# cmp-nct/ggllm.cpp

Hardware: NVIDIA B200
Metric: falcon40b_q4_k_decode_tokens_per_s (higher is better)
Workload: dtype int8 x int4 block dots (dp4a), fp32 accumulate; f32 KV/attention

## Files before the change

### ggllm.cpp_b200/csrc/bwtest.cu

```cuda
#include "common.cuh"
__global__ void __launch_bounds__(256) read_kernel(const uint4 * __restrict__ p, size_t n, int unroll_dummy, unsigned * out) {
    unsigned acc = 0;
    const size_t stride = (size_t) gridDim.x * blockDim.x;
    size_t i = (size_t) blockIdx.x * blockDim.x + threadIdx.x;
    for (; i + 7 * stride < n; i += 8 * stride) {
        uint4 v[8];
#pragma unroll
        for (int u = 0; u < 8; u++) v[u] = ldg_stream_v4(p + i + u * stride);
#pragma unroll
        for (int u = 0; u < 8; u++) acc += v[u].x ^ v[u].y ^ v[u].z ^ v[u].w;
    }
    for (; i < n; i += stride) { const uint4 v = ldg_stream_v4(p + i); acc += v.x ^ v.y ^ v.z ^ v.w; }
    if (acc == 0x12345678u && unroll_dummy) *out = acc;
}
extern "C" float b200_read_bandwidth_gbs(size_t bytes, int ctas_per_sm) {
    void * p = nullptr; unsigned * o = nullptr;
    B200_CUDA_CHECK(cudaMalloc(&p, bytes)); B200_CUDA_CHECK(cudaMalloc(&o, 4));
    B200_CUDA_CHECK(cudaMemset(p, 1, bytes));
    int dev, sms; cudaGetDevice(&dev); cudaDeviceGetAttribute(&sms, cudaDevAttrMultiProcessorCount, dev);
    cudaEvent_t e0, e1; cudaEventCreate(&e0); cudaEventCreate(&e1);
    float best = 0.f;
    for (int it = 0; it < 6; it++) {
        cudaEventRecord(e0);
        read_kernel<<<sms * ctas_per_sm, 256>>>((const uint4 *) p, bytes / 16, 0, o);
        cudaEventRecord(e1); cudaEventSynchronize(e1);
        float ms; cudaEventElapsedTime(&ms, e0, e1);
        const float g = (float) (bytes / 1e6 / ms);
        if (it > 0 && g > best) best = g;
    }
    cudaFree(p); cudaFree(o);
    return best;
}
```

### ggllm.cpp_b200/csrc/common.cuh

```cuda
#pragma once
#include <cuda_runtime.h>
#include <cuda_fp16.h>
#include <cstdint>
#include <cstdio>
#include <cstdlib>

#define B200_CUDA_CHECK(expr)                                                                        \
    do {                                                                                             \
        cudaError_t err_ = (expr);                                                                   \
        if (err_ != cudaSuccess) {                                                                   \
            fprintf(stderr, "b200: CUDA error %d (%s) at %s:%d: %s\n", (int) err_,                   \
                    cudaGetErrorString(err_), __FILE__, __LINE__, #expr);                            \
            exit(1);                                                                                 \
        }                                                                                            \
    } while (0)

#define B200_ASSERT(x)                                                                               \
    do {                                                                                             \
        if (!(x)) {                                                                                  \
            fprintf(stderr, "B200_ASSERT: %s:%d: %s\n", __FILE__, __LINE__, #x);                     \
            abort();                                                                                 \
        }                                                                                            \
    } while (0)

enum : int {
    T_F32 = 0, T_F16 = 1, T_Q4_0 = 2, T_Q4_1 = 3, T_Q5_0 = 6, T_Q5_1 = 7, T_Q8_0 = 8, T_Q8_1 = 9,
    T_Q2_K = 10, T_Q3_K = 11, T_Q4_K = 12, T_Q5_K = 13, T_Q6_K = 14, T_Q8_K = 15,
};

static inline size_t round_up(size_t v, size_t a) { return (v + a - 1) / a * a; }

#define B200_CARVEOUT 25

#ifdef __CUDACC__

__device__ __forceinline__ uint4 ldg_stream_v4(const void * p) {
    uint4 r;
    asm volatile("ld.global.nc.L1::no_allocate.v4.u32 {%0,%1,%2,%3}, [%4];"
                 : "=r"(r.x), "=r"(r.y), "=r"(r.z), "=r"(r.w) : "l"(p));
    return r;
}
__device__ __forceinline__ uint2 ldg_stream_v2(const void * p) {
    uint2 r;
    asm volatile("ld.global.nc.L1::no_allocate.v2.u32 {%0,%1}, [%2];" : "=r"(r.x), "=r"(r.y) : "l"(p));
    return r;
}
__device__ __forceinline__ uint32_t ldg_stream_u32(const void * p) {
    uint32_t r;
    asm volatile("ld.global.nc.L1::no_allocate.u32 %0, [%1];" : "=r"(r) : "l"(p));
    return r;
}
__device__ __forceinline__ uint4 ldg_v4(const void * p) { return __ldg(reinterpret_cast<const uint4 *>(p)); }
__device__ __forceinline__ uint32_t ldg_u32(const void * p) { return __ldg(reinterpret_cast<const uint32_t *>(p)); }
__device__ __forceinline__ uint16_t ldg_u16(const void * p) { return __ldg(reinterpret_cast<const uint16_t *>(p)); }

__device__ __forceinline__ float f16_bits_to_f32(uint16_t h) { return __half2float(__ushort_as_half(h)); }
__device__ __forceinline__ uint16_t f32_to_f16_bits(float f) { return __half_as_ushort(__float2half_rn(f)); }

__device__ __forceinline__ float warp_sum(float v) {
#pragma unroll
    for (int o = 16; o > 0; o >>= 1) v += __shfl_xor_sync(0xffffffffu, v, o);
    return v;
}
__device__ __forceinline__ float warp_max(float v) {
#pragma unroll
    for (int o = 16; o > 0; o >>= 1) v = fmaxf(v, __shfl_xor_sync(0xffffffffu, v, o));
    return v;
}
__device__ __forceinline__ double warp_sum_d(double v) {
#pragma unroll
    for (int o = 16; o > 0; o >>= 1) v += __shfl_xor_sync(0xffffffffu, v, o);
    return v;
}

__device__ __forceinline__ int dp4a_ss(int a, int b, int c) { return __dp4a(a, b, c); }
__device__ __forceinline__ int dp4a_us(unsigned a, int b, int c) {
    int d;
    asm("dp4a.u32.s32 %0, %1, %2, %3;" : "=r"(d) : "r"(a), "r"(b), "r"(c));
    return d;
}

__device__ __forceinline__ uint32_t smem_u32(const void * p) { return (uint32_t) __cvta_generic_to_shared(p); }
__device__ __forceinline__ void mbar_init(uint64_t * bar, uint32_t count) {
    asm volatile("mbarrier.init.shared::cta.b64 [%0], %1;" :: "r"(smem_u32(bar)), "r"(count));
}
__device__ __forceinline__ void mbar_fence_init() { asm volatile("fence.mbarrier_init.release.cluster;" ::: "memory"); }
__device__ __forceinline__ void mbar_expect_tx(uint64_t * bar, uint32_t bytes) {
    asm volatile("mbarrier.arrive.expect_tx.shared::cta.b64 _, [%0], %1;" :: "r"(smem_u32(bar)), "r"(bytes) : "memory");
}
__device__ __forceinline__ void mbar_wait(uint64_t * bar, uint32_t phase) {
    asm volatile(
        "{\n\t.reg .pred p;\n\t"
        "WAIT_%=:\n\t"
        "mbarrier.try_wait.parity.shared::cta.b64 p, [%0], %1;\n\t"
        "@p bra DONE_%=;\n\t"
        "bra WAIT_%=;\n\t"
        "DONE_%=:\n\t}"
        :: "r"(smem_u32(bar)), "r"(phase) : "memory");
}
__device__ __forceinline__ void tma_load_1d(void * smem_dst, const void * gmem_src, uint32_t bytes, uint64_t * bar) {
    asm volatile("cp.async.bulk.shared::cluster.global.mbarrier::complete_tx::bytes [%0], [%1], %2, [%3];"
                 :: "r"(smem_u32(smem_dst)), "l"(gmem_src), "r"(bytes), "r"(smem_u32(bar)) : "memory");
}

__device__ __forceinline__ unsigned long long gtimer() { unsigned long long t; asm volatile("mov.u64 %0, %globaltimer;" : "=l"(t)); return t; }
__device__ __forceinline__ void trace_begin(unsigned long long * slot) { if (slot && threadIdx.x == 0) atomicMin(slot, gtimer()); }
__device__ __forceinline__ void trace_end(unsigned long long * slot) { if (slot && threadIdx.x == 0) atomicMax(slot + 1, gtimer()); }

#endif

unsigned long long * b200_trace_slot(const char * name);
```

### ggllm.cpp_b200/csrc/kernels.h

```cpp
#pragma once
#include "formats.cuh"

size_t wplanes_layout(WPlanes & W, int type, int K, int M);
void   wplanes_upload(WPlanes & W, int type, int K, int M, const void * host_raw, cudaStream_t stream);
void   wplanes_from_device_raw(WPlanes & W, int type, int K, int M, const void * dev_raw, cudaStream_t stream);
void   wplanes_alloc_random(WPlanes & W, int type, int K, int M, uint64_t seed, cudaStream_t stream);
void   launch_repack_rows(const WPlanes & W, const void * stage_dev, int64_t row0, int64_t nrows, cudaStream_t stream);
void   wplanes_free(WPlanes & W);
void   launch_dequant_rows(const WPlanes & W, const int32_t * rows_dev, int nrows, float * dst, int64_t dst_stride, cudaStream_t stream);

size_t actq_bytes(int act_type, int K, int N);
void   actq_bind(ActQ & A, int act_type, int K, int N, void * base);
void   launch_quantize_act(const float * x, int64_t x_stride, const ActQ & A, cudaStream_t stream);
void   launch_actq_to_f16(const ActQ & A, __half * dst, int64_t dst_stride, cudaStream_t stream);

enum { EPI_NONE = 0, EPI_GELU = 1, EPI_ADD2 = 2 };
struct MmvEpilogue { int kind; const float * r1; const float * r2;
    const ActQ * qout; unsigned * qctr;
    int late_wait; };
void   launch_mmv(const WPlanes & W, const ActQ & A, float * y, int64_t y_stride, MmvEpilogue epi, cudaStream_t stream);
void   launch_mmv_f(const WPlanes & W, const float * x, int64_t x_stride, int N, float * y, int64_t y_stride, cudaStream_t stream);

struct FastX {
    int mode;
    int N;
    ActQ A;
    const float * x; int64_t x_stride;
    const float * ra, * rb;
    const float * gamma, * beta;
    float * x_out;
    int l2_dist;
};
bool   launch_mmv_fast_x(const WPlanes & W, const FastX & X, float * y, int64_t y_stride, MmvEpilogue e, cudaStream_t stream);
bool   mmv_fast_supports(int wtype, int K, int mode);
bool   mmv_fast_fills_sm(const WPlanes & W);
void   launch_layernorm(const float * x, int64_t x_stride, const float * g, const float * b, float * y, int64_t y_stride,
                        int n, int rows, cudaStream_t stream);
void   launch_argmax(const float * x, int n, int32_t * out_a, int32_t * out_b, cudaStream_t stream);
void   launch_argmax_hist(const float * x, int n, int32_t * out, int32_t * hist, int * step, cudaStream_t stream);
void   launch_layernorm_q(float * x, int64_t x_stride, const float * ra, const float * rb, int64_t r_stride,
                          const float * g1, const float * b1, const ActQ * A1,
                          const float * g2, const float * b2, const ActQ * A2, int n, int rows, cudaStream_t stream);
void   launch_gelu(const float * x, float * y, int64_t n, cudaStream_t stream);
void   launch_f32_to_f16(const float * x, __half * y, int64_t n, cudaStream_t stream);
void   launch_add(const float * a, const float * b, float * y, int64_t n, cudaStream_t stream);
void   launch_add3(const float * a, const float * b, const float * c, float * y, int64_t n, cudaStream_t stream);
void   launch_mul_bcast(const float * a, const float * b, float * y, int64_t n, int64_t nb, cudaStream_t stream);
void   launch_add_bcast(const float * a, const float * b, float * y, int64_t n, int64_t nb, cudaStream_t stream);
void   launch_scale(const float * a, float s, float * y, int64_t n, cudaStream_t stream);
struct RopeParams { int n_past; int head_dim; float theta_scale; };
float  rope_theta_scale_host(int head_dim, int n_ctx_rope, int dynamic_mode, float ntk_alpha, int freq_base);
void   launch_rope_neox(float * x, int n_tok, int n_head, int head_dim, int64_t tok_stride, int n_past, const int * n_past_dev,
                        float theta_scale, cudaStream_t stream);

struct AttnParams {
    int n_head, n_head_kv, head_dim;
    int n_tok;
    int n_past;
    const int * n_past_dev;
    int n_ctx;
    int64_t qkv_stride;
    unsigned long long * trace;
    const ActQ * qout;
    __half * k16; __half * vt16;
    int fuse_rope; float rope_theta_scale;
    int long_ctx;
};
int    attention_long_threshold();
void   launch_rope_kv_append(float * qkv, float * k_cache, float * v_cache, const AttnParams & p, float theta_scale, cudaStream_t stream);
int    launch_attention(const float * qkv, const float * k_cache, const float * v_cache, float * out, int64_t out_stride,
                        const AttnParams & p, float * scratch, cudaStream_t stream);
size_t attention_scratch_bytes(const AttnParams & p);
bool   launch_attention_ws(const float * qkv, float * out, int64_t out_stride, const AttnParams & p, cudaStream_t stream);
int    attention_ctx_pad(int n_ctx);
size_t attention_shadow_halves(int n_head_kv, int n_ctx);
void   launch_kv_shadow_refresh(const float * k_cache, const float * v_cache, __half * k16, __half * vt16, int n_head_kv, int n_ctx, int pos, int n, cudaStream_t stream);
size_t attention_prefill_scratch_bytes(int n_head, int n_tok, int T);
void   launch_attention_prefill(const float * qkv, const float * k_cache, const float * v_cache, float * out, int64_t out_stride,
                                const AttnParams & p, float * scratch, cudaStream_t stream);

void   launch_mmq_gemm(const WPlanes & W, const __half * X, int64_t x_stride, int N, float * Y, int64_t y_stride,
                       int epi_gelu, void * workspace, size_t workspace_bytes, cudaStream_t stream);
size_t mmq_gemm_workspace_bytes(const WPlanes & W, int N);

#define B200_SAMPLER_MAX_WINDOW 256
struct SamplerParams { int top_k; float top_p; float temp; float repeat_penalty; };
struct SamplerState;
SamplerState * sampler_state_alloc();
void   sampler_state_free(SamplerState * s);
void   launch_sampler_init(SamplerState * s, uint32_t seed, const int32_t * window_dev, int n, int cap, cudaStream_t stream);
void   launch_sample(const float * logits, int n_vocab, const SamplerParams & p, SamplerState * st, float * work, int32_t * out, int32_t * hist, int * step, cudaStream_t stream);

struct b200_falcon;
bool   falcon_adopt_matrix(b200_falcon * f, const char * ggcc_name, const WPlanes & W);
int    falcon_eval_begin(b200_falcon * f, const int32_t * tokens, int n_tokens, int n_past, int n_ctx_rope, int all_logits);
void   falcon_eval_finish(b200_falcon * f, float * logits);
```

### ggllm.cpp_b200/csrc/mmv_fast.cu

```cuda
#include "kernels.h"

#include "mmv_fast.cuh"

template <int TYPE, int NT, int J, int D, int MODE>
__device__ __forceinline__ void mmv_body(const WPlanes & W, const FastX & X, float * __restrict__ y, int64_t y_stride, const Epi & epi,
                                         const int cta, const int nctas, const int n, uint8_t * smem) {
    using T = FX<TYPE>;
    constexpr int NW = NT / 32;
    uint64_t * bar = reinterpret_cast<uint64_t *>(smem);
    float * partial = reinterpret_cast<float *>(smem + 16);
    double * red = reinterpret_cast<double *>(smem + 16 + 2 * NW * 4 * 4);
    int8_t * xq = reinterpret_cast<int8_t *>(smem + ((16 + 2 * NW * 4 * 4 + NW * 8 + 15) & ~15));
    const int tid = threadIdx.x, lane = tid & 31, warp = tid >> 5;
    const int P = W.nb * T::PPB;
    const ActQ & A = X.A;

    trace_begin(epi.trace);
    if (tid == 0 && MODE == 0) { mbar_init(bar, 1); mbar_fence_init(); }
    const int per = W.M / nctas, rem = W.M % nctas;
    const int row0 = cta * per + min(cta, rem), row1 = row0 + per + (cta < rem ? 1 : 0);
    const int nrows = row1 - row0;

    int gidx[J]; bool valid[J];
    WP wp[J];
    int aux[J];
#pragma unroll
    for (int j = 0; j < J; j++) { const int g = j * NT + tid; valid[j] = g < P; gidx[j] = valid[j] ? g : P - 1; wp[j] = T::wp(W, gidx[j]); aux[j] = piece_aux<TYPE>(gidx[j]); }

    typename T::WR w[D][J];
    ring_fill<TYPE, J, D>(w, wp, row0, row1);
    const L2PF pf = l2pf_of(W, X.l2_dist);
    if (pf.dist > 0 && tid == 0) l2_prefetch_rows(pf, min(row0 + D, row1), min(row0 + D + pf.dist, row1));

    if (!epi.late_wait) asm volatile("griddepcontrol.wait;" ::: "memory");
    typename T::XR xr[J];
    if (MODE == 0) {
        if (tid == 0) {
            mbar_expect_tx(bar, (uint32_t) W.K);
            tma_load_1d(xq, A.q + (size_t) n * W.K, (uint32_t) W.K, bar);
        }
        __syncthreads();
        mbar_wait(bar, 0);
#pragma unroll
        for (int j = 0; j < J; j++) xr[j] = valid[j] ? T::load_x(xq, A, n, gidx[j]) : zero_xr<TYPE>();
    } else if constexpr (T::HAS_PROLOGUE_QUANT) {
        const float * xrow = X.x + (size_t) n * X.x_stride;
        float mean = 0.f, scale = 1.f;
#pragma unroll
        for (int j = 0; j < J; j++) {
            int ea, eb; T::seg(gidx[j], ea, eb);
            float v[32];
#pragma unroll
            for (int i = 0; i < 4; i++) {
                const float4 a = *reinterpret_cast<const float4 *>(xrow + ea + 4 * i), b = *reinterpret_cast<const float4 *>(xrow + eb + 4 * i);
                v[4 * i] = a.x; v[4 * i + 1] = a.y; v[4 * i + 2] = a.z; v[4 * i + 3] = a.w;
                v[16 + 4 * i] = b.x; v[17 + 4 * i] = b.y; v[18 + 4 * i] = b.z; v[19 + 4 * i] = b.w;
            }
            if (MODE == 2 && J == 1) {
                if (X.ra) {
                    const float * ra = X.ra + (size_t) n * X.x_stride, * rb = X.rb + (size_t) n * X.x_stride;
#pragma unroll
                    for (int i = 0; i < 16; i++) { v[i] = __fadd_rn(__fadd_rn(ra[ea + i], rb[ea + i]), v[i]); v[16 + i] = __fadd_rn(__fadd_rn(ra[eb + i], rb[eb + i]), v[16 + i]); }
                }
                if (X.x_out && cta == 0 && valid[j]) {
                    float * xo = X.x_out + (size_t) n * X.x_stride;
#pragma unroll
                    for (int i = 0; i < 16; i++) { xo[ea + i] = v[i]; xo[eb + i] = v[16 + i]; }
                }
                double s = 0.0;
                if (valid[j]) {
#pragma unroll
                    for (int i = 0; i < 32; i++) s += (double) v[i];
                }
                s = warp_sum_d(s);
                if (lane == 0) red[warp] = s;
                __syncthreads();
                double t = 0.0;
#pragma unroll
                for (int wi = 0; wi < NW; wi++) t += red[wi];
                mean = (float) (t / W.K);
                __syncthreads();
                double s2 = 0.0;
                if (valid[j]) {
#pragma unroll
                    for (int i = 0; i < 32; i++) { const float c = __fsub_rn(v[i], mean); s2 += (double) __fmul_rn(c, c); }
                }
                s2 = warp_sum_d(s2);
                if (lane == 0) red[warp] = s2;
                __syncthreads();
                t = 0.0;
#pragma unroll
                for (int wi = 0; wi < NW; wi++) t += red[wi];
                scale = __fdiv_rn(1.0f, __fsqrt_rn(__fadd_rn((float) (t / W.K), 1e-5f)));
#pragma unroll
                for (int i = 0; i < 16; i++) {
                    v[i] = __fadd_rn(__fmul_rn(__fmul_rn(__fsub_rn(v[i], mean), scale), X.gamma[ea + i]), X.beta[ea + i]);
                    v[16 + i] = __fadd_rn(__fmul_rn(__fmul_rn(__fsub_rn(v[16 + i], mean), scale), X.gamma[eb + i]), X.beta[eb + i]);
                }
            }
            if (!valid[j]) {
#pragma unroll
                for (int i = 0; i < 32; i++) v[i] = 0.f;
            }
            xr[j] = T::quant_x(v, gidx[j], lane);
        }
        __syncthreads();
    }

    int gcount = 0;
    const int ekind = epi.kind; const float * r1p = epi.r1, * r2p = epi.r2;
    ring_run<TYPE, NT, J, D, false>(w, wp, row0, row1, wp, 0, 0, xr, aux, partial, gcount, 0, tid,
        [&](int row, float v) {
            if (ekind == EPI_GELU) v = gelu_lut(v);
            else if (ekind == EPI_ADD2) v = (v + r1p[(size_t) n * y_stride + row]) + r2p[(size_t) n * y_stride + row];
            y[(size_t) n * y_stride + row] = v;
        },
        [&]() { asm volatile("griddepcontrol.launch_dependents;" ::: "memory"); }, pf);
    if (epi.late_wait) asm volatile("griddepcontrol.wait;" ::: "memory");
    if (epi.qctr) {
        __shared__ int s_do;
        __threadfence();
        __syncthreads();
        if (nrows > 0) {
            for (int b = row0 >> 8; b <= (row1 - 1) >> 8; b++) {
                if (tid == 0) {
                    const unsigned cnt = (unsigned) (min(row1, (b + 1) << 8) - max(row0, b << 8));
                    const unsigned old = atomicAdd(epi.qctr + b, cnt);
                    s_do = old + cnt == 256u;
                    if (s_do) epi.qctr[b] = 0;
                }
                __syncthreads();
                if (s_do && warp == 0) {
                    __threadfence();
                    const float * src = y + (size_t) n * y_stride + (b << 8) + lane * 8;
                    const float4 p = __ldcg(reinterpret_cast<const float4 *>(src)), q = __ldcg(reinterpret_cast<const float4 *>(src) + 1);
                    const float v[8] = { p.x, p.y, p.z, p.w, q.x, q.y, q.z, q.w };
                    if (epi.qA.type == T_Q8_K) quantize_chunk8<T_Q8_K>(v, lane, epi.qA, n, (b << 8) + lane * 8);
                    else quantize_chunk8<T_Q8_0>(v, lane, epi.qA, n, (b << 8) + lane * 8);
                }
                __syncthreads();
            }
        }
    }
    trace_end(epi.trace);
}

template <int TYPE, int NT, int J, int D, int MODE>
__global__ void __launch_bounds__(NT) __maxnreg__(NT <= 256 ? 96 : 128) mmv_fast_kernel(const WPlanes W, const FastX X, float * __restrict__ y, int64_t y_stride, const Epi epi) {
    extern __shared__ __align__(16) uint8_t smem[];
    mmv_body<TYPE, NT, J, D, MODE>(W, X, y, y_stride, epi, (int) blockIdx.x, (int) gridDim.x, (int) blockIdx.y, smem);
}

static int fast_num_sms() {
    static int n = 0;
    if (!n) { int dev; B200_CUDA_CHECK(cudaGetDevice(&dev)); B200_CUDA_CHECK(cudaDeviceGetAttribute(&n, cudaDevAttrMultiProcessorCount, dev)); }
    return n;
}

template <int TYPE, int NT, int J, int D, int MODE>
static void launch_mode(const WPlanes & W, const FastX & X, float * y, int64_t y_stride, Epi epi, cudaStream_t stream) {
    const size_t smem = ((16 + 2 * (NT / 32) * 4 * 4 + (NT / 32) * 8 + 15) & ~15) + (size_t) ((W.K + 15) & ~15);
    static bool set = false;
    if (!set) { B200_CUDA_CHECK(cudaFuncSetAttribute(mmv_fast_kernel<TYPE, NT, J, D, MODE>, cudaFuncAttributeMaxDynamicSharedMemorySize, 100 * 1024));
        B200_CUDA_CHECK(cudaFuncSetAttribute(mmv_fast_kernel<TYPE, NT, J, D, MODE>, cudaFuncAttributePreferredSharedMemoryCarveout, B200_CARVEOUT)); set = true; }
    int ctas = fast_num_sms() * (NT == 128 ? 4 : NT == 160 || NT == 192 ? 3 : NT == 256 ? 2 : 1);
    if (ctas > (W.M + 3) / 4) ctas = (W.M + 3) / 4;
    cudaLaunchConfig_t cfg{};
    cfg.gridDim = dim3((unsigned) ctas, (unsigned) X.N); cfg.blockDim = dim3(NT); cfg.dynamicSmemBytes = smem; cfg.stream = stream;
    cudaLaunchAttribute attr[1];
    attr[0].id = cudaLaunchAttributeProgrammaticStreamSerialization;
    attr[0].val.programmaticStreamSerializationAllowed = 1;
    cfg.attrs = attr; cfg.numAttrs = getenv("B200_NO_PDL") ? 0 : 1;
    B200_CUDA_CHECK(cudaLaunchKernelEx(&cfg, mmv_fast_kernel<TYPE, NT, J, D, MODE>, W, X, y, y_stride, epi));
}
template <int TYPE, int NT, int J, int D>
static void launch_cfg(const WPlanes & W, const FastX & X, float * y, int64_t y_stride, Epi epi, cudaStream_t stream) {
    if (X.mode == 0) launch_mode<TYPE, NT, J, D, 0>(W, X, y, y_stride, epi, stream);
    else if constexpr (FX<TYPE>::HAS_PROLOGUE_QUANT) {
        if (X.mode == 1) launch_mode<TYPE, NT, J, D, 1>(W, X, y, y_stride, epi, stream);
        else if (J == 1) launch_mode<TYPE, NT, J, D, J == 1 ? 2 : 1>(W, X, y, y_stride, epi, stream);
        else B200_ASSERT(!"mmv_fast: LayerNorm prologue needs J == 1");
    } else B200_ASSERT(!"mmv_fast: this weight type takes quantised activations only (mode 0)");
}

template <int TYPE>
static bool launch_type(const WPlanes & W, const FastX & X, float * y, int64_t y_stride, Epi epi, cudaStream_t stream) {
    const int P = W.nb * FX<TYPE>::PPB;
    if (W.K > 64 * 1024) return false;
    if (X.mode == 2 && P > 512) return false;
    constexpr int D1 = FX<TYPE>::D256;
    if (P <= 128 && D1 == 4) launch_cfg<TYPE, 128, 1, D1>(W, X, y, y_stride, epi, stream);
    else if (P > 128 && P <= 160 && D1 == 8 && !getenv("B200_NO_NT160")) launch_cfg<TYPE, 160, 1, D1>(W, X, y, y_stride, epi, stream);
    else if (P <= 256) launch_cfg<TYPE, 256, 1, D1>(W, X, y, y_stride, epi, stream);
    else if (P > 256 && P <= 512 && D1 == 8 && X.mode == 0 && !getenv("B200_NO_NT256J2")) launch_cfg<TYPE, 256, 2, D1 / 2>(W, X, y, y_stride, epi, stream);
    else if (P <= 512) launch_cfg<TYPE, 512, 1, D1>(W, X, y, y_stride, epi, stream);
    else if (P > 512 && P <= 576 && D1 == 8 && X.mode == 0 && !getenv("B200_NO_NT192")) launch_cfg<TYPE, 192, 3, 2>(W, X, y, y_stride, epi, stream);
    else if (P <= 1024) launch_cfg<TYPE, 512, 2, D1 / 2>(W, X, y, y_stride, epi, stream);
    else if (P <= 2048 && D1 == 8) launch_cfg<TYPE, 512, 4, 2>(W, X, y, y_stride, epi, stream);
    else return false;
    return true;
}

bool launch_mmv_fast_x(const WPlanes & W, const FastX & X, float * y, int64_t y_stride, MmvEpilogue e, cudaStream_t stream) {
    const char * nm = W.M > 40000 ? "mmv_lmhead" : W.K > 16384 ? "mmv_down" : W.M > 16384 ? "mmv_up" : W.M > 8192 ? "mmv_qkv" : "mmv_wo";
    Epi epi = { e.kind, e.r1, e.r2, b200_trace_slot(nm), ActQ{}, nullptr, getenv("B200_NO_LATE_WAIT") ? 0 : e.late_wait };
    if (e.qout && e.qctr) {
        B200_ASSERT(X.N == 1 && W.M % 256 == 0 && e.qout->K == W.M && (e.qout->type == T_Q8_K || e.qout->type == T_Q8_0));
        epi.qA = *e.qout; epi.qctr = e.qctr;
    }
    static int dist_bytes = -1;
    if (dist_bytes < 0) { const char * s = getenv("B200_L2PF_KB"); dist_bytes = (s ? atoi(s) : 0) * 1024; }
    FastX Xp = X;
    Xp.l2_dist = W.stride[0] ? (int) (dist_bytes / W.stride[0]) : 0;
    switch (W.type) {
        case T_Q4_K: return launch_type<T_Q4_K>(W, Xp, y, y_stride, epi, stream);
        case T_Q4_0: return launch_type<T_Q4_0>(W, Xp, y, y_stride, epi, stream);
        case T_Q3_K: return X.mode == 0 && !getenv("B200_Q3K_GENERIC") && launch_type<T_Q3_K>(W, Xp, y, y_stride, epi, stream);
    }
    return false;
}
bool mmv_fast_supports(int wtype, int K, int mode) {
    if (wtype != T_Q4_K && wtype != T_Q4_0) return false;
    const int P = wtype == T_Q4_K ? K / 32 : K / 32;
    return K <= 64 * 1024 && P <= (mode == 2 ? 512 : 2048);
}
bool mmv_fast_fills_sm(const WPlanes & W) {
    if ((W.type != T_Q4_K && W.type != T_Q4_0) || getenv("B200_NO_NT192")) return false;
    const int P = W.K / 32;
    return P > 512 && P <= 576;
}
bool launch_mmv_fast(const WPlanes & W, const ActQ & A, float * y, int64_t y_stride, MmvEpilogue e, cudaStream_t stream) {
    FastX X{}; X.mode = 0; X.A = A; X.N = A.N;
    return launch_mmv_fast_x(W, X, y, y_stride, e, stream);
}
```

### ggllm.cpp_b200/csrc/mmv_fast.cuh

```cuda
#pragma once
#include "kernels.h"
#include "actquant.cuh"

struct Epi { int kind; const float * r1; const float * r2; unsigned long long * trace; ActQ qA; unsigned * qctr; int late_wait; };


__device__ __forceinline__ int dot16(const uint32_t w0, const uint32_t w1, const uint32_t w2, const uint32_t w3, const uint4 x) {
    int s = dp4a_us(w0, (int) x.x, 0); s = dp4a_us(w1, (int) x.y, s); s = dp4a_us(w2, (int) x.z, s); return dp4a_us(w3, (int) x.w, s);
}
__device__ __forceinline__ int dp2a_lo_su(int pair16, uint32_t bytes) { int d; asm("dp2a.lo.s32.u32 %0, %1, %2, %3;" : "=r"(d) : "r"(pair16), "r"(bytes), "r"(0)); return d; }
__device__ __forceinline__ int dp2a_hi_su(int pair16, uint32_t bytes) { int d; asm("dp2a.hi.s32.u32 %0, %1, %2, %3;" : "=r"(d) : "r"(pair16), "r"(bytes), "r"(0)); return d; }
__device__ __forceinline__ int dp2a_lo_ss(int pair16, uint32_t bytes, int c) { int d; asm("dp2a.lo.s32.s32 %0, %1, %2, %3;" : "=r"(d) : "r"(pair16), "r"(bytes), "r"(c)); return d; }
__device__ __forceinline__ int dp2a_hi_ss(int pair16, uint32_t bytes, int c) { int d; asm("dp2a.hi.s32.s32 %0, %1, %2, %3;" : "=r"(d) : "r"(pair16), "r"(bytes), "r"(c)); return d; }
__device__ __forceinline__ float gelu_lut(float v) {
    const float f = __half2float(__float2half_rn(v));
    const float g = 0.5f * f * (1.0f + tanhf(0.79788456080286535587989211986876f * f * (1.0f + 0.044715f * f * f)));
    return __half2float(__float2half_rn(g));
}

struct WP { const uint8_t * b0, * b1, * b2, * b3; uint32_t s0, s1, s2, s3; };
__device__ __forceinline__ const uint8_t * opaque_ptr(const uint8_t * p) { unsigned long long v = (unsigned long long) p; asm volatile("" : "+l"(v)); return (const uint8_t *) v; }

template <int TYPE> struct FX;

template <> struct FX<T_Q4_K> {
    static constexpr int PPB = 8;
    static constexpr bool HAS_PROLOGUE_QUANT = true;
    static constexpr int D256 = 8;
    struct XR { uint4 xl, xh; int bs; float xd; };
    struct WR { uint4 q; uint32_t sm, dd; };
    __device__ static XR load_x(const int8_t * xq, const ActQ & A, int n, int g) {
        const int b = g >> 3, pc = g & 7, p = pc >> 1, half = pc & 1;
        XR r;
        const int e0 = b * 256 + 64 * p + 16 * half;
        r.xl = *reinterpret_cast<const uint4 *>(xq + e0);
        r.xh = *reinterpret_cast<const uint4 *>(xq + e0 + 32);
        const int16_t * bs = A.bs + (size_t) n * (A.K / 16) + b * 16 + 4 * p + half;
        r.bs = ((int) bs[0] & 0xffff) | ((int) bs[2] << 16);
        r.xd = A.d[(size_t) n * (A.K / 256) + b];
        return r;
    }
    __device__ static void seg(int g, int & ea, int & eb) { const int b = g >> 3, pc = g & 7; ea = b * 256 + 64 * (pc >> 1) + 16 * (pc & 1); eb = ea + 32; }
    __device__ static XR quant_x(const float (&v)[32], int g, int lane) {
        int ea, eb; seg(g, ea, eb);
        float amax = 0.f, vmax = 0.f; int imax = 0;
#pragma unroll
        for (int i = 0; i < 32; i++) { const float ax = fabsf(v[i]); const int idx = (i < 16 ? ea : eb - 16) + i; if (ax > amax || (ax == amax && ax > 0.f && idx < imax)) { amax = ax; vmax = v[i]; imax = idx; } }
#pragma unroll
        for (int o = 1; o < 8; o <<= 1) {
            const float oa = __shfl_xor_sync(0xffffffffu, amax, o), ov = __shfl_xor_sync(0xffffffffu, vmax, o);
            const int oi = __shfl_xor_sync(0xffffffffu, imax, o);
            if (oa > amax || (oa == amax && oi < imax)) { amax = oa; vmax = ov; imax = oi; }
        }
        XR r;
        const bool zero = amax == 0.f;
        const float iscale = zero ? 0.f : __fdiv_rn(-128.f, vmax);
        r.xd = zero ? 0.f : __fdiv_rn(1.f, iscale);
        int s0 = 0, s1 = 0;
        uint32_t w[8];
#pragma unroll
        for (int i = 0; i < 8; i++) {
            uint32_t pk = 0;
#pragma unroll
            for (int k = 0; k < 4; k++) {
                const int q = zero ? 0 : min(127, __float2int_rn(__fmul_rn(iscale, v[4 * i + k])));
                if (i < 4) s0 += q; else s1 += q;
                pk |= (uint32_t) (q & 0xff) << (8 * k);
            }
            w[i] = pk;
        }
        r.xl = make_uint4(w[0], w[1], w[2], w[3]); r.xh = make_uint4(w[4], w[5], w[6], w[7]);
        r.bs = (s0 & 0xffff) | (s1 << 16);
        (void) lane;
        return r;
    }
    __device__ static WP wp(const WPlanes & W, int g) {
        WP r; r.b0 = opaque_ptr(W.p[0] + (size_t) g * 16); r.b1 = opaque_ptr(W.p[1] + (size_t) (g >> 1) * 4); r.b2 = opaque_ptr(W.p[2] + (size_t) (g >> 3) * 4);
        r.s0 = W.stride[0]; r.s1 = W.stride[1]; r.s2 = W.stride[2];
        return r;
    }
    __device__ static WR load_w(const WP & p, uint32_t row) {
        WR r;
        r.q = ldg_stream_v4(p.b0 + (uint64_t) row * p.s0);
        r.sm = ldg_u32(p.b1 + (uint64_t) row * p.s1);
        r.dd = ldg_u32(p.b2 + (uint64_t) row * p.s2);
        return r;
    }
    __device__ static float dot(const WR & w, const XR & x) {
        const int il = dot16(w.q.x & 0x0F0F0F0F, w.q.y & 0x0F0F0F0F, w.q.z & 0x0F0F0F0F, w.q.w & 0x0F0F0F0F, x.xl);
        const int ih = dot16(w.q.x & 0xF0F0F0F0, w.q.y & 0xF0F0F0F0, w.q.z & 0xF0F0F0F0, w.q.w & 0xF0F0F0F0, x.xh) >> 4;
        const int isum = dp2a_lo_su((il & 0xffff) | (ih << 16), w.sm);
        const int msum = dp2a_hi_su(x.bs, w.sm);
        const float2 dm = __half22float2(*reinterpret_cast<const __half2 *>(&w.dd));
        return (dm.x * x.xd) * (float) isum - (dm.y * x.xd) * (float) msum;
    }
};

template <> struct FX<T_Q4_0> {
    static constexpr int PPB = 1;
    static constexpr bool HAS_PROLOGUE_QUANT = true;
    static constexpr int D256 = 8;
    struct XR { uint4 xl, xh; int bs; float xd; };
    struct WR { uint4 q; uint32_t d; };
    __device__ static XR load_x(const int8_t * xq, const ActQ & A, int n, int g) {
        XR r;
        r.xl = *reinterpret_cast<const uint4 *>(xq + g * 32);
        r.xh = *reinterpret_cast<const uint4 *>(xq + g * 32 + 16);
        r.bs = A.bs[(size_t) n * (A.K / 32) + g];
        r.xd = A.d[(size_t) n * (A.K / 32) + g];
        return r;
    }
    __device__ static void seg(int g, int & ea, int & eb) { ea = g * 32; eb = ea + 16; }
    __device__ static XR quant_x(const float (&v)[32], int, int) {
        float amax = 0.f;
#pragma unroll
        for (int i = 0; i < 32; i++) amax = fmaxf(amax, fabsf(v[i]));
        const float id = amax != 0.f ? __fdiv_rn(127.f, amax) : 0.f;
        XR r;
        r.xd = __half2float(__float2half_rn(__fdiv_rn(amax, 127.f)));
        int s = 0;
        uint32_t w[8];
#pragma unroll
        for (int i = 0; i < 8; i++) {
            uint32_t pk = 0;
#pragma unroll
            for (int k = 0; k < 4; k++) { const int q = __float2int_rn(__fmul_rn(v[4 * i + k], id)); s += q; pk |= (uint32_t) (q & 0xff) << (8 * k); }
            w[i] = pk;
        }
        r.xl = make_uint4(w[0], w[1], w[2], w[3]); r.xh = make_uint4(w[4], w[5], w[6], w[7]);
        r.bs = s;
        return r;
    }
    __device__ static WP wp(const WPlanes & W, int g) {
        WP r; r.b0 = opaque_ptr(W.p[0] + (size_t) g * 16); r.b1 = opaque_ptr(W.p[1] + (size_t) g * 2); r.b2 = nullptr;
        r.s0 = W.stride[0]; r.s1 = W.stride[1]; r.s2 = 0;
        return r;
    }
    __device__ static WR load_w(const WP & p, uint32_t row) {
        WR r;
        r.q = ldg_stream_v4(p.b0 + (uint64_t) row * p.s0);
        r.d = ldg_u16(p.b1 + (uint64_t) row * p.s1);
        return r;
    }
    __device__ static float dot(const WR & w, const XR & x) {
        int s = dot16(w.q.x & 0x0F0F0F0F, w.q.y & 0x0F0F0F0F, w.q.z & 0x0F0F0F0F, w.q.w & 0x0F0F0F0F, x.xl);
        s += dot16(w.q.x & 0xF0F0F0F0, w.q.y & 0xF0F0F0F0, w.q.z & 0xF0F0F0F0, w.q.w & 0xF0F0F0F0, x.xh) >> 4;
        s -= 8 * x.bs;
        return ((float) s * f16_bits_to_f32((uint16_t) w.d)) * x.xd;
    }
};

template <> struct FX<T_Q3_K> {
    static constexpr int PPB = 4;
    static constexpr bool HAS_PROLOGUE_QUANT = false;
    static constexpr int D256 = 4;
    struct XR { uint4 x[4]; int bsA, bsB; float xd; };
    struct WR { uint4 q, hm; uint32_t sc, d; };
    __device__ static XR load_x(const int8_t * xq, const ActQ & A, int n, int g) {
        const int b = g >> 2, pc = g & 3, hn = pc >> 1, c = pc & 1;
        XR r;
        const int16_t * bs = A.bs + (size_t) n * (A.K / 16) + b * 16 + 8 * hn + c;
#pragma unroll
        for (int quad = 0; quad < 4; quad++) r.x[quad] = *reinterpret_cast<const uint4 *>(xq + b * 256 + 128 * hn + 32 * quad + 16 * c);
        r.bsA = ((int) bs[0] & 0xffff) | ((int) bs[2] << 16);
        r.bsB = ((int) bs[4] & 0xffff) | ((int) bs[6] << 16);
        r.xd = A.d[(size_t) n * (A.K / 256) + b];
        return r;
    }
    __device__ static void seg(int, int & ea, int & eb) { ea = 0; eb = 0; }
    __device__ static XR quant_x(const float (&)[32], int, int) { return XR{}; }
    __device__ static WP wp(const WPlanes & W, int g) {
        WP r;
        r.b0 = opaque_ptr(W.p[0] + (size_t) g * 16); r.b1 = opaque_ptr(W.p[1] + (size_t) (g >> 2) * 32 + (g & 1) * 16);
        r.b2 = opaque_ptr(W.p[2] + (size_t) g * 4);  r.b3 = opaque_ptr(W.p[3] + (size_t) (g >> 2) * 2);
        r.s0 = W.stride[0]; r.s1 = W.stride[1]; r.s2 = W.stride[2]; r.s3 = W.stride[3];
        return r;
    }
    __device__ static WR load_w(const WP & p, uint32_t row) {
        WR r;
        r.q = ldg_stream_v4(p.b0 + (uint64_t) row * p.s0);
        r.hm = ldg_v4(p.b1 + (uint64_t) row * p.s1);
        r.sc = ldg_u32(p.b2 + (uint64_t) row * p.s2);
        r.d = ldg_u16(p.b3 + (uint64_t) row * p.s3);
        return r;
    }
    __device__ static float dot(const WR & w, const XR & x, int hsh) {
        const uint32_t q[4] = { w.q.x, w.q.y, w.q.z, w.q.w }, hm[4] = { w.hm.x, w.hm.y, w.hm.z, w.hm.w };
        const uint32_t hbase = 0x01010101u << hsh;
        int i[4];
#pragma unroll
        for (int quad = 0; quad < 4; quad++) {
            const uint32_t qm = 0x03030303u << (2 * quad), hmk = hbase << quad;
            const int dq = dot16(q[0] & qm, q[1] & qm, q[2] & qm, q[3] & qm, x.x[quad]);
            const int dh = dot16(hm[0] & hmk, hm[1] & hmk, hm[2] & hmk, hm[3] & hmk, x.x[quad]);
            i[quad] = (dq >> (2 * quad)) + ((dh >> (hsh + quad)) << 2);
        }
        int isum = dp2a_lo_ss((i[0] & 0xffff) | (i[1] << 16), w.sc, 0);
        isum = dp2a_hi_ss((i[2] & 0xffff) | (i[3] << 16), w.sc, isum);
        int bsum = dp2a_lo_ss(x.bsA, w.sc, 0);
        bsum = dp2a_hi_ss(x.bsB, w.sc, bsum);
        return (f16_bits_to_f32((uint16_t) w.d) * x.xd) * (float) (isum - 4 * bsum);
    }
};

template <int G> __device__ __forceinline__ float transpose_reduce(const float (&acc)[G], int lane, int & row_of_lane) {
    float w;
    if (G == 4) {
        const bool hi = lane & 16;
        float v0 = hi ? acc[2] : acc[0], v1 = hi ? acc[3] : acc[1];
        v0 += __shfl_xor_sync(0xffffffffu, hi ? acc[0] : acc[2], 16);
        v1 += __shfl_xor_sync(0xffffffffu, hi ? acc[1] : acc[3], 16);
        const bool mid = lane & 8;
        w = mid ? v1 : v0;
        w += __shfl_xor_sync(0xffffffffu, mid ? v0 : v1, 8);
        w += __shfl_xor_sync(0xffffffffu, w, 4);
        row_of_lane = (hi ? 2 : 0) + (mid ? 1 : 0);
    } else if (G == 2) {
        const bool hi = lane & 16;
        w = hi ? acc[G - 1] : acc[0];
        w += __shfl_xor_sync(0xffffffffu, hi ? acc[0] : acc[G - 1], 16);
        w += __shfl_xor_sync(0xffffffffu, w, 8);
        w += __shfl_xor_sync(0xffffffffu, w, 4);
        row_of_lane = hi ? 1 : 0;
    } else {
        w = acc[0];
        w += __shfl_xor_sync(0xffffffffu, w, 16);
        w += __shfl_xor_sync(0xffffffffu, w, 8);
        w += __shfl_xor_sync(0xffffffffu, w, 4);
        row_of_lane = 0;
    }
    w += __shfl_xor_sync(0xffffffffu, w, 2);
    w += __shfl_xor_sync(0xffffffffu, w, 1);
    return w;
}


struct L2PF { const uint8_t * p[3]; uint32_t s[3]; int dist; };
__device__ __forceinline__ void l2_prefetch_rows(const L2PF & pf, int a, int b) {
    if (b <= a) return;
#pragma unroll
    for (int i = 0; i < 3; i++) {
        if (!pf.p[i]) continue;
        const uint8_t * src = pf.p[i] + (size_t) a * pf.s[i];
        const uint32_t bytes = (uint32_t) (b - a) * pf.s[i];
        asm volatile("cp.async.bulk.prefetch.L2.global [%0], %1;" :: "l"(src), "r"(bytes) : "memory");
    }
}
__device__ __forceinline__ L2PF l2pf_of(const WPlanes & W, int dist) {
    L2PF r; r.dist = dist;
#pragma unroll
    for (int i = 0; i < 3; i++) { r.p[i] = W.p[i]; r.s[i] = W.stride[i]; }
    return r;
}

__device__ __forceinline__ void named_sync(int id, int n) { asm volatile("bar.sync %0, %1;" :: "r"(id), "r"(n) : "memory"); }

template <int TYPE> __device__ __forceinline__ int piece_aux(int g) { return TYPE == T_Q3_K ? 4 * ((g & 3) >> 1) : 0; }
template <int TYPE> __device__ __forceinline__ float piece_dot(const typename FX<TYPE>::WR & w, const typename FX<TYPE>::XR & x, int aux) {
    if constexpr (TYPE == T_Q3_K) return FX<TYPE>::dot(w, x, aux); else return FX<TYPE>::dot(w, x);
}
template <int TYPE> __device__ __forceinline__ typename FX<TYPE>::XR zero_xr() {
    typename FX<TYPE>::XR r{}; return r;
}

template <int TYPE, int J, int D>
__device__ __forceinline__ void ring_fill(typename FX<TYPE>::WR (&w)[D][J], const WP (&wp)[J], int r0, int r1) {
    if (r1 <= r0) return;
#pragma unroll
    for (int s = 0; s < D; s++) {
        const uint32_t row = (uint32_t) min(r0 + s, r1 - 1);
#pragma unroll
        for (int j = 0; j < J; j++) w[s][j] = FX<TYPE>::load_w(wp[j], row);
    }
}

template <int TYPE, int NTG, int J, int D, bool CHECKED, bool HASNEXT, class Store>
__device__ __forceinline__ void ring_pass(typename FX<TYPE>::WR (&w)[D][J], const WP (&wp)[J], const int r0, const int nrows, const int npad, const int base,
                                          const WP (&wpn)[J], const int n0, const int n1,
                                          const typename FX<TYPE>::XR (&xr)[J], const int (&aux)[J], float * partial, int & gcount, const int bar_id, const int tg, Store & store) {
    using T = FX<TYPE>;
    constexpr int NWG = NTG / 32, G = (D % 4 == 0) ? 4 : (D % 2 == 0) ? 2 : 1;
    const int lane = tg & 31, warp = tg >> 5;
    float acc[G];
#pragma unroll
    for (int s = 0; s < D; s++) {
        float a = piece_dot<TYPE>(w[s][0], xr[0], aux[0]);
#pragma unroll
        for (int j = 1; j < J; j++) a += piece_dot<TYPE>(w[s][j], xr[j], aux[j]);
        acc[s % G] = a;
        const int nxt = base + D + s;
        if (!CHECKED || nxt < nrows) {
#pragma unroll
            for (int j = 0; j < J; j++) w[s][j] = T::load_w(wp[j], (uint32_t) (r0 + nxt));
        } else if (HASNEXT && nxt >= npad && n1 > n0) {
            const uint32_t k = (uint32_t) min(n0 + nxt - npad, n1 - 1);
#pragma unroll
            for (int j = 0; j < J; j++) w[s][j] = T::load_w(wpn[j], k);
        }
        if ((s % G) == G - 1) {
            const int gi = (base + s) / G;
            int rl;
            const float v0 = transpose_reduce<G>(acc, lane, rl);
            float * part = partial + (gcount & 1) * NWG * G;
            gcount++;
            if ((lane & (G == 4 ? 7 : G == 2 ? 15 : 31)) == 0) part[warp * G + rl] = v0;
            named_sync(bar_id, NTG);
            if (tg < G) {
                const int row = r0 + gi * G + tg;
                if (!CHECKED || row < r0 + nrows) {
                    float v = 0.f;
#pragma unroll
                    for (int wi = 0; wi < NWG; wi++) v += part[wi * G + tg];
                    store(row, v);
                }
            }
        }
    }
}

template <int TYPE, int NTG, int J, int D, bool HASNEXT, class Store, class Tail>
__device__ __forceinline__ void ring_run(typename FX<TYPE>::WR (&w)[D][J], const WP (&wp)[J], const int r0, const int r1,
                                         const WP (&wpn)[J], const int n0, const int n1,
                                         const typename FX<TYPE>::XR (&xr)[J], const int (&aux)[J], float * partial, int & gcount, const int bar_id, const int tg,
                                         Store store, Tail before_tail, const L2PF pf = L2PF{ { nullptr, nullptr, nullptr }, { 0, 0, 0 }, 0 }) {
    const int nrows = r1 - r0, npad = (nrows + D - 1) / D * D;
    if (npad == 0) { before_tail(); if (HASNEXT) ring_fill<TYPE, J, D>(w, wpn, n0, n1); return; }
    int base = 0;
    for (; base + 2 * D <= nrows; base += D) {
        if (pf.dist > 0 && tg == 0) l2_prefetch_rows(pf, min(r0 + base + D + pf.dist, r1), min(r0 + base + 2 * D + pf.dist, r1));
        ring_pass<TYPE, NTG, J, D, false, false>(w, wp, r0, nrows, npad, base, wpn, n0, n1, xr, aux, partial, gcount, bar_id, tg, store);
    }
    before_tail();
    for (; base < npad; base += D)
        ring_pass<TYPE, NTG, J, D, true, HASNEXT>(w, wp, r0, nrows, npad, base, wpn, n0, n1, xr, aux, partial, gcount, bar_id, tg, store);
}
```

Measured before the change: 211.7.

## Stream weight rows into shared memory via TMA bulk-copy ring in mmv_fast

Replaces the register-ring per-thread global loads (plus L2 bulk prefetch) for Q4_K/Q4_0 matrix-vector kernels with a multi-stage shared-memory ring filled by cp.async.bulk, with mbarrier completion and thread 0 issuing the next stage after a named barrier. Stage size and stage count are chosen per launch from the shared-memory carveout, which is raised from 25 to 72 to make room. The aim is to keep more bytes in flight per SM for a bandwidth-bound decode. The cost is higher shared-memory use, which can limit occupancy, plus a single-thread issue point and barrier latency. A bulk-read bandwidth test is also added.

```diff
diff --git a/ggllm.cpp_b200/csrc/bwtest.cu b/ggllm.cpp_b200/csrc/bwtest.cu
--- a/ggllm.cpp_b200/csrc/bwtest.cu
+++ b/ggllm.cpp_b200/csrc/bwtest.cu
@@ -31,3 +31,61 @@
     cudaFree(p); cudaFree(o);
     return best;
 }
+
+__global__ void __launch_bounds__(288) read_bulk_kernel(const uint8_t * __restrict__ p, size_t nchunks, uint32_t stage, int nstage, unsigned * out) {
+    extern __shared__ __align__(128) uint8_t sm[];
+    uint64_t * full = reinterpret_cast<uint64_t *>(sm), * empty = full + 16;
+    uint8_t * ring = sm + 256;
+    constexpr int NCW = 8;
+    const int tid = threadIdx.x, warp = tid >> 5;
+    if (tid == 0) { for (int s = 0; s < nstage; s++) { mbar_init(full + s, 1); mbar_init(empty + s, NCW); } mbar_fence_init(); }
+    __syncthreads();
+    const size_t nmine = nchunks > blockIdx.x ? (nchunks - blockIdx.x + gridDim.x - 1) / gridDim.x : 0;
+    if (warp == NCW) {
+        if ((tid & 31) == 0) {
+            for (size_t k = 0; k < nmine; k++) {
+                const int s = (int) (k % nstage);
+                if (k >= (size_t) nstage) mbar_wait(empty + s, (uint32_t) ((k / nstage - 1) & 1));
+                mbar_expect_tx(full + s, stage);
+                tma_load_1d(ring + (size_t) s * stage, p + (blockIdx.x + k * gridDim.x) * (size_t) stage, stage, full + s);
+            }
+        }
+        return;
+    }
+    unsigned acc = 0;
+    for (size_t k = 0; k < nmine; k++) {
+        const int s = (int) (k % nstage);
+        mbar_wait(full + s, (uint32_t) ((k / nstage) & 1));
+        const uint4 * st = reinterpret_cast<const uint4 *>(ring + (size_t) s * stage);
+        for (uint32_t i = tid; i < stage / 16; i += NCW * 32) { const uint4 v = st[i]; acc += v.x ^ v.y ^ v.z ^ v.w; }
+        __syncwarp();
+        if ((tid & 31) == 0) mbar_arrive(empty + s);
+    }
+    if (acc == 0x12345678u && out) *out = acc;
+}
+extern "C" float b200_read_bandwidth_bulk_gbs(size_t bytes, int kb_in_flight, int stage_kb) {
+    const uint32_t stage = (uint32_t) stage_kb * 1024;
+    const int nstage = kb_in_flight / stage_kb;
+    if (nstage < 1 || nstage > 16) return 0.f;
+    const size_t nchunks = bytes / stage;
+    void * p = nullptr; unsigned * o = nullptr;
+    B200_CUDA_CHECK(cudaMalloc(&p, nchunks * stage)); B200_CUDA_CHECK(cudaMalloc(&o, 4));
+    B200_CUDA_CHECK(cudaMemset(p, 1, nchunks * stage));
+    int dev, sms; cudaGetDevice(&dev); cudaDeviceGetAttribute(&sms, cudaDevAttrMultiProcessorCount, dev);
+    const size_t smem = 256 + (size_t) nstage * stage;
+    B200_CUDA_CHECK(cudaFuncSetAttribute(read_bulk_kernel, cudaFuncAttributeMaxDynamicSharedMemorySize, (int) smem));
+    cudaEvent_t e0, e1; cudaEventCreate(&e0); cudaEventCreate(&e1);
+    float best = 0.f;
+    for (int it = 0; it < 6; it++) {
+        cudaEventRecord(e0);
+        read_bulk_kernel<<<sms, 288, smem>>>((const uint8_t *) p, nchunks, stage, nstage, o);
+        cudaEventRecord(e1); cudaEventSynchronize(e1);
+        B200_CUDA_CHECK(cudaGetLastError());
+        float ms; cudaEventElapsedTime(&ms, e0, e1);
+        const float g = (float) (nchunks * stage / 1e6 / ms);
+        if (it > 0 && g > best) best = g;
+    }
+    cudaEventDestroy(e0); cudaEventDestroy(e1);
+    cudaFree(p); cudaFree(o);
+    return best;
+}
diff --git a/ggllm.cpp_b200/csrc/common.cuh b/ggllm.cpp_b200/csrc/common.cuh
--- a/ggllm.cpp_b200/csrc/common.cuh
+++ b/ggllm.cpp_b200/csrc/common.cuh
@@ -30,7 +30,7 @@
 
 static inline size_t round_up(size_t v, size_t a) { return (v + a - 1) / a * a; }
 
-#define B200_CARVEOUT 25
+#define B200_CARVEOUT 72
 
 #ifdef __CUDACC__
 
@@ -88,6 +88,9 @@
 __device__ __forceinline__ void mbar_expect_tx(uint64_t * bar, uint32_t bytes) {
     asm volatile("mbarrier.arrive.expect_tx.shared::cta.b64 _, [%0], %1;" :: "r"(smem_u32(bar)), "r"(bytes) : "memory");
 }
+__device__ __forceinline__ void mbar_arrive(uint64_t * bar) {
+    asm volatile("mbarrier.arrive.shared::cta.b64 _, [%0];" :: "r"(smem_u32(bar)) : "memory");
+}
 __device__ __forceinline__ void mbar_wait(uint64_t * bar, uint32_t phase) {
     asm volatile(
         "{\n\t.reg .pred p;\n\t"
diff --git a/ggllm.cpp_b200/csrc/kernels.h b/ggllm.cpp_b200/csrc/kernels.h
--- a/ggllm.cpp_b200/csrc/kernels.h
+++ b/ggllm.cpp_b200/csrc/kernels.h
@@ -29,7 +29,7 @@
     const float * ra, * rb;
     const float * gamma, * beta;
     float * x_out;
-    int l2_dist;
+    int nstage, stage_rows;
 };
 bool   launch_mmv_fast_x(const WPlanes & W, const FastX & X, float * y, int64_t y_stride, MmvEpilogue e, cudaStream_t stream);
 bool   mmv_fast_supports(int wtype, int K, int mode);
diff --git a/ggllm.cpp_b200/csrc/mmv_fast.cu b/ggllm.cpp_b200/csrc/mmv_fast.cu
--- a/ggllm.cpp_b200/csrc/mmv_fast.cu
+++ b/ggllm.cpp_b200/csrc/mmv_fast.cu
@@ -1,36 +1,63 @@
+#include <algorithm>
+
 #include "kernels.h"
 
 #include "mmv_fast.cuh"
 
-template <int TYPE, int NT, int J, int D, int MODE>
+struct MmvSmem { int partial, red, xq, ring; };
+__host__ __device__ inline MmvSmem mmv_smem(int nw, int K) {
+    MmvSmem m;
+    m.partial = 8 + 8 * RING_MAX_STAGES;
+    m.red = m.partial + 2 * nw * 4 * 4;
+    m.xq = (m.red + nw * 8 + 15) & ~15;
+    m.ring = (m.xq + ((K + 15) & ~15) + 127) & ~127;
+    return m;
+}
+
+template <int TYPE, int NT, int J, int R, int MODE>
 __device__ __forceinline__ void mmv_body(const WPlanes & W, const FastX & X, float * __restrict__ y, int64_t y_stride, const Epi & epi,
                                          const int cta, const int nctas, const int n, uint8_t * smem) {
     using T = FX<TYPE>;
     constexpr int NW = NT / 32;
+    constexpr bool BULK = TYPE != T_Q3_K;
+    const MmvSmem L = mmv_smem(NW, W.K);
     uint64_t * bar = reinterpret_cast<uint64_t *>(smem);
-    float * partial = reinterpret_cast<float *>(smem + 16);
-    double * red = reinterpret_cast<double *>(smem + 16 + 2 * NW * 4 * 4);
-    int8_t * xq = reinterpret_cast<int8_t *>(smem + ((16 + 2 * NW * 4 * 4 + NW * 8 + 15) & ~15));
+    uint64_t * full = bar + 1;
+    float * partial = reinterpret_cast<float *>(smem + L.partial);
+    double * red = reinterpret_cast<double *>(smem + L.red);
+    int8_t * xq = reinterpret_cast<int8_t *>(smem + L.xq);
+    const uint32_t ring = smem_u32(smem + L.ring);
     const int tid = threadIdx.x, lane = tid & 31, warp = tid >> 5;
     const int P = W.nb * T::PPB;
     const ActQ & A = X.A;
 
     trace_begin(epi.trace);
-    if (tid == 0 && MODE == 0) { mbar_init(bar, 1); mbar_fence_init(); }
     const int per = W.M / nctas, rem = W.M % nctas;
     const int row0 = cta * per + min(cta, rem), row1 = row0 + per + (cta < rem ? 1 : 0);
     const int nrows = row1 - row0;
+    const int rs = X.stage_rows, ns = X.nstage, nst = BULK ? (nrows + rs - 1) / rs : 0;
+    uint32_t stage_bytes = 0;
+#pragma unroll
+    for (int i = 0; i < (BULK ? T::NPL : 0); i++) stage_bytes += rs * W.stride[i];
+    if (tid == 0) {
+        if (MODE == 0) mbar_init(bar, 1);
+        if (BULK) for (int s = 0; s < ns; s++) mbar_init(full + s, 1);
+        mbar_fence_init();
+        if constexpr (BULK) for (int k = 0; k < min(ns, nst); k++) stage_issue<TYPE>(W, ring + k * stage_bytes, full + k, row0 + k * rs, min(rs, nrows - k * rs), rs);
+    }
 
     int gidx[J]; bool valid[J];
+    int aux[J];
+#pragma unroll
+    for (int j = 0; j < J; j++) { const int g = j * NT + tid; valid[j] = g < P; gidx[j] = valid[j] ? g : P - 1; aux[j] = piece_aux<TYPE>(gidx[j]); }
+    constexpr int D = BULK ? 1 : R;
     WP wp[J];
-    int aux[J];
-#pragma unroll
-    for (int j = 0; j < J; j++) { const int g = j * NT + tid; valid[j] = g < P; gidx[j] = valid[j] ? g : P - 1; wp[j] = T::wp(W, gidx[j]); aux[j] = piece_aux<TYPE>(gidx[j]); }
-
     typename T::WR w[D][J];
-    ring_fill<TYPE, J, D>(w, wp, row0, row1);
-    const L2PF pf = l2pf_of(W, X.l2_dist);
-    if (pf.dist > 0 && tid == 0) l2_prefetch_rows(pf, min(row0 + D, row1), min(row0 + D + pf.dist, row1));
+    if constexpr (!BULK) {
+#pragma unroll
+        for (int j = 0; j < J; j++) wp[j] = T::wp(W, gidx[j]);
+        ring_fill<TYPE, J, D>(w, wp, row0, row1);
+    }
 
     if (!epi.late_wait) asm volatile("griddepcontrol.wait;" ::: "memory");
     typename T::XR xr[J];
@@ -107,15 +134,56 @@
         __syncthreads();
     }
 
-    int gcount = 0;
     const int ekind = epi.kind; const float * r1p = epi.r1, * r2p = epi.r2;
-    ring_run<TYPE, NT, J, D, false>(w, wp, row0, row1, wp, 0, 0, xr, aux, partial, gcount, 0, tid,
-        [&](int row, float v) {
-            if (ekind == EPI_GELU) v = gelu_lut(v);
-            else if (ekind == EPI_ADD2) v = (v + r1p[(size_t) n * y_stride + row]) + r2p[(size_t) n * y_stride + row];
-            y[(size_t) n * y_stride + row] = v;
-        },
-        [&]() { asm volatile("griddepcontrol.launch_dependents;" ::: "memory"); }, pf);
+    auto store = [&](int row, float v) {
+        if (ekind == EPI_GELU) v = gelu_lut(v);
+        else if (ekind == EPI_ADD2) v = (v + r1p[(size_t) n * y_stride + row]) + r2p[(size_t) n * y_stride + row];
+        y[(size_t) n * y_stride + row] = v;
+    };
+    auto trigger = [&]() { asm volatile("griddepcontrol.launch_dependents;" ::: "memory"); };
+    if constexpr (BULK) {
+        SP sp[J];
+#pragma unroll
+        for (int j = 0; j < J; j++) sp[j] = stage_ptrs<TYPE>(W, gidx[j], rs);
+        if (nst <= ns) trigger();
+        int slot = 0, grp = 0; uint32_t phase = 0;
+        for (int k = 0; k < nst; k++) {
+            const uint32_t st = ring + slot * stage_bytes;
+            mbar_wait(full + slot, phase);
+            for (int q = 0; q < rs && k * rs + q < nrows; q += R, grp++) {
+                float acc[R];
+#pragma unroll
+                for (int r = 0; r < R; r++) {
+                    float a = piece_dot<TYPE>(stage_load<TYPE>(st, sp[0], q + r), xr[0], aux[0]);
+#pragma unroll
+                    for (int j = 1; j < J; j++) a += piece_dot<TYPE>(stage_load<TYPE>(st, sp[j], q + r), xr[j], aux[j]);
+                    acc[r] = a;
+                }
+                int rl;
+                const float v0 = transpose_reduce<R>(acc, lane, rl);
+                float * part = partial + (grp & 1) * NW * R;
+                if ((lane & (R == 4 ? 7 : R == 2 ? 15 : 31)) == 0) part[warp * R + rl] = v0;
+                named_sync(0, NT);
+                if (q + R == rs && k + ns < nst) {
+                    if (tid == 0) stage_issue<TYPE>(W, st, full + slot, row0 + (k + ns) * rs, min(rs, nrows - (k + ns) * rs), rs);
+                    if (k + ns == nst - 1) trigger();
+                }
+                if (tid < R) {
+                    const int row = row0 + k * rs + q + tid;
+                    if (row < row1) {
+                        float v = 0.f;
+#pragma unroll
+                        for (int wi = 0; wi < NW; wi++) v += part[wi * R + tid];
+                        store(row, v);
+                    }
+                }
+            }
+            if (++slot == ns) { slot = 0; phase ^= 1; }
+        }
+    } else {
+        int gcount = 0;
+        ring_run<TYPE, NT, J, D>(w, wp, row0, row1, xr, aux, partial, gcount, 0, tid, store, trigger);
+    }
     if (epi.late_wait) asm volatile("griddepcontrol.wait;" ::: "memory");
     if (epi.qctr) {
         __shared__ int s_do;
@@ -145,10 +213,10 @@
     trace_end(epi.trace);
 }
 
-template <int TYPE, int NT, int J, int D, int MODE>
+template <int TYPE, int NT, int J, int R, int MODE>
 __global__ void __launch_bounds__(NT) __maxnreg__(NT <= 256 ? 96 : 128) mmv_fast_kernel(const WPlanes W, const FastX X, float * __restrict__ y, int64_t y_stride, const Epi epi) {
-    extern __shared__ __align__(16) uint8_t smem[];
-    mmv_body<TYPE, NT, J, D, MODE>(W, X, y, y_stride, epi, (int) blockIdx.x, (int) gridDim.x, (int) blockIdx.y, smem);
+    extern __shared__ __align__(128) uint8_t smem[];
+    mmv_body<TYPE, NT, J, R, MODE>(W, X, y, y_stride, epi, (int) blockIdx.x, (int) gridDim.x, (int) blockIdx.y, smem);
 }
 
 static int fast_num_sms() {
@@ -157,13 +225,38 @@
     return n;
 }
 
-template <int TYPE, int NT, int J, int D, int MODE>
+#define MMV_STAGE_KB 32
+#define MMV_RING_KB 128
+#define MMV_SIDE_KB 24
+static int env_kb(const char * name, int dflt) { const char * s = getenv(name); return s ? atoi(s) : dflt; }
+
+template <int TYPE, int NT, int J, int R, int MODE>
 static void launch_mode(const WPlanes & W, const FastX & X, float * y, int64_t y_stride, Epi epi, cudaStream_t stream) {
-    const size_t smem = ((16 + 2 * (NT / 32) * 4 * 4 + (NT / 32) * 8 + 15) & ~15) + (size_t) ((W.K + 15) & ~15);
-    static bool set = false;
-    if (!set) { B200_CUDA_CHECK(cudaFuncSetAttribute(mmv_fast_kernel<TYPE, NT, J, D, MODE>, cudaFuncAttributeMaxDynamicSharedMemorySize, 100 * 1024));
-        B200_CUDA_CHECK(cudaFuncSetAttribute(mmv_fast_kernel<TYPE, NT, J, D, MODE>, cudaFuncAttributePreferredSharedMemoryCarveout, B200_CARVEOUT)); set = true; }
-    int ctas = fast_num_sms() * (NT == 128 ? 4 : NT == 160 || NT == 192 ? 3 : NT == 256 ? 2 : 1);
+    constexpr int CPS = NT == 128 ? 4 : NT == 160 || NT == 192 ? 3 : NT == 256 ? 2 : 1;
+    static const size_t stage_target = (size_t) env_kb("B200_MMV_STAGE_KB", MMV_STAGE_KB) * 1024, ring_target = (size_t) env_kb("B200_MMV_RING_KB", MMV_RING_KB) * 1024;
+    const MmvSmem L = mmv_smem(NT / 32, W.K);
+    FastX Xs = X;
+    size_t smem = (size_t) L.xq + (size_t) ((W.K + 15) & ~15);
+    if (TYPE != T_Q3_K) {
+        size_t row_bytes = 0;
+        for (int i = 0; i < FX<TYPE>::NPL; i++) row_bytes += W.stride[i];
+        const bool side = CPS > 1 && NT != 192;
+        const size_t carve = (size_t) B200_CARVEOUT * 228 * 1024 / 100 - (side ? MMV_SIDE_KB * 1024 : 0);
+        const size_t fit = carve / CPS > (size_t) L.ring + 1024 ? carve / CPS - L.ring - 1024 : 0;
+        const size_t avail = std::min(fit, ring_target / CPS);
+        int rs = std::max<int>(R, (int) ((stage_target + row_bytes / 2) / row_bytes) / R * R);
+        while (rs > R && 2 * rs * row_bytes > avail) rs -= R;
+        const size_t stage = rs * row_bytes;
+        Xs.stage_rows = rs;
+        Xs.nstage = (int) std::max<size_t>(2, std::min<size_t>(avail / stage, RING_MAX_STAGES));
+        smem = (size_t) L.ring + Xs.nstage * stage;
+    }
+    B200_ASSERT(smem <= 227 * 1024);
+    static size_t smem_set = 0;
+    if (!smem_set)
+        B200_CUDA_CHECK(cudaFuncSetAttribute(mmv_fast_kernel<TYPE, NT, J, R, MODE>, cudaFuncAttributePreferredSharedMemoryCarveout, B200_CARVEOUT));
+    if (smem > smem_set) { B200_CUDA_CHECK(cudaFuncSetAttribute(mmv_fast_kernel<TYPE, NT, J, R, MODE>, cudaFuncAttributeMaxDynamicSharedMemorySize, (int) smem)); smem_set = smem; }
+    int ctas = fast_num_sms() * CPS;
     if (ctas > (W.M + 3) / 4) ctas = (W.M + 3) / 4;
     cudaLaunchConfig_t cfg{};
     cfg.gridDim = dim3((unsigned) ctas, (unsigned) X.N); cfg.blockDim = dim3(NT); cfg.dynamicSmemBytes = smem; cfg.stream = stream;
@@ -171,14 +264,14 @@
     attr[0].id = cudaLaunchAttributeProgrammaticStreamSerialization;
     attr[0].val.programmaticStreamSerializationAllowed = 1;
     cfg.attrs = attr; cfg.numAttrs = getenv("B200_NO_PDL") ? 0 : 1;
-    B200_CUDA_CHECK(cudaLaunchKernelEx(&cfg, mmv_fast_kernel<TYPE, NT, J, D, MODE>, W, X, y, y_stride, epi));
-}
-template <int TYPE, int NT, int J, int D>
+    B200_CUDA_CHECK(cudaLaunchKernelEx(&cfg, mmv_fast_kernel<TYPE, NT, J, R, MODE>, W, Xs, y, y_stride, epi));
+}
+template <int TYPE, int NT, int J, int R>
 static void launch_cfg(const WPlanes & W, const FastX & X, float * y, int64_t y_stride, Epi epi, cudaStream_t stream) {
-    if (X.mode == 0) launch_mode<TYPE, NT, J, D, 0>(W, X, y, y_stride, epi, stream);
+    if (X.mode == 0) launch_mode<TYPE, NT, J, R, 0>(W, X, y, y_stride, epi, stream);
     else if constexpr (FX<TYPE>::HAS_PROLOGUE_QUANT) {
-        if (X.mode == 1) launch_mode<TYPE, NT, J, D, 1>(W, X, y, y_stride, epi, stream);
-        else if (J == 1) launch_mode<TYPE, NT, J, D, J == 1 ? 2 : 1>(W, X, y, y_stride, epi, stream);
+        if (X.mode == 1) launch_mode<TYPE, NT, J, R, 1>(W, X, y, y_stride, epi, stream);
+        else if (J == 1) launch_mode<TYPE, NT, J, R, J == 1 ? 2 : 1>(W, X, y, y_stride, epi, stream);
         else B200_ASSERT(!"mmv_fast: LayerNorm prologue needs J == 1");
     } else B200_ASSERT(!"mmv_fast: this weight type takes quantised activations only (mode 0)");
 }
@@ -188,17 +281,24 @@
     const int P = W.nb * FX<TYPE>::PPB;
     if (W.K > 64 * 1024) return false;
     if (X.mode == 2 && P > 512) return false;
-    constexpr int D1 = FX<TYPE>::D256;
-    if (P <= 128 && D1 == 4) launch_cfg<TYPE, 128, 1, D1>(W, X, y, y_stride, epi, stream);
-    else if (P > 128 && P <= 160 && D1 == 8 && !getenv("B200_NO_NT160")) launch_cfg<TYPE, 160, 1, D1>(W, X, y, y_stride, epi, stream);
-    else if (P <= 256) launch_cfg<TYPE, 256, 1, D1>(W, X, y, y_stride, epi, stream);
-    else if (P > 256 && P <= 512 && D1 == 8 && X.mode == 0 && !getenv("B200_NO_NT256J2")) launch_cfg<TYPE, 256, 2, D1 / 2>(W, X, y, y_stride, epi, stream);
-    else if (P <= 512) launch_cfg<TYPE, 512, 1, D1>(W, X, y, y_stride, epi, stream);
-    else if (P > 512 && P <= 576 && D1 == 8 && X.mode == 0 && !getenv("B200_NO_NT192")) launch_cfg<TYPE, 192, 3, 2>(W, X, y, y_stride, epi, stream);
-    else if (P <= 1024) launch_cfg<TYPE, 512, 2, D1 / 2>(W, X, y, y_stride, epi, stream);
-    else if (P <= 2048 && D1 == 8) launch_cfg<TYPE, 512, 4, 2>(W, X, y, y_stride, epi, stream);
-    else return false;
-    return true;
+    if constexpr (TYPE == T_Q3_K) {
+        if (P <= 128) launch_cfg<TYPE, 128, 1, 4>(W, X, y, y_stride, epi, stream);
+        else if (P <= 256) launch_cfg<TYPE, 256, 1, 4>(W, X, y, y_stride, epi, stream);
+        else if (P <= 512) launch_cfg<TYPE, 512, 1, 4>(W, X, y, y_stride, epi, stream);
+        else if (P <= 1024) launch_cfg<TYPE, 512, 2, 2>(W, X, y, y_stride, epi, stream);
+        else return false;
+        return true;
+    } else {
+        if (P > 128 && P <= 160 && !getenv("B200_NO_NT160")) launch_cfg<TYPE, 160, 1, 2>(W, X, y, y_stride, epi, stream);
+        else if (P <= 256) launch_cfg<TYPE, 256, 1, 2>(W, X, y, y_stride, epi, stream);
+        else if (P <= 512 && X.mode == 0 && !getenv("B200_NO_NT256J2")) launch_cfg<TYPE, 256, 2, 2>(W, X, y, y_stride, epi, stream);
+        else if (P <= 512) launch_cfg<TYPE, 512, 1, 2>(W, X, y, y_stride, epi, stream);
+        else if (P <= 576 && X.mode == 0 && !getenv("B200_NO_NT192")) launch_cfg<TYPE, 192, 3, 1>(W, X, y, y_stride, epi, stream);
+        else if (P <= 1024) launch_cfg<TYPE, 512, 2, 1>(W, X, y, y_stride, epi, stream);
+        else if (P <= 2048) launch_cfg<TYPE, 512, 4, 1>(W, X, y, y_stride, epi, stream);
+        else return false;
+        return true;
+    }
 }
 
 bool launch_mmv_fast_x(const WPlanes & W, const FastX & X, float * y, int64_t y_stride, MmvEpilogue e, cudaStream_t stream) {
@@ -208,14 +308,10 @@
         B200_ASSERT(X.N == 1 && W.M % 256 == 0 && e.qout->K == W.M && (e.qout->type == T_Q8_K || e.qout->type == T_Q8_0));
         epi.qA = *e.qout; epi.qctr = e.qctr;
     }
-    static int dist_bytes = -1;
-    if (dist_bytes < 0) { const char * s = getenv("B200_L2PF_KB"); dist_bytes = (s ? atoi(s) : 0) * 1024; }
-    FastX Xp = X;
-    Xp.l2_dist = W.stride[0] ? (int) (dist_bytes / W.stride[0]) : 0;
     switch (W.type) {
-        case T_Q4_K: return launch_type<T_Q4_K>(W, Xp, y, y_stride, epi, stream);
-        case T_Q4_0: return launch_type<T_Q4_0>(W, Xp, y, y_stride, epi, stream);
-        case T_Q3_K: return X.mode == 0 && !getenv("B200_Q3K_GENERIC") && launch_type<T_Q3_K>(W, Xp, y, y_stride, epi, stream);
+        case T_Q4_K: return launch_type<T_Q4_K>(W, X, y, y_stride, epi, stream);
+        case T_Q4_0: return launch_type<T_Q4_0>(W, X, y, y_stride, epi, stream);
+        case T_Q3_K: return X.mode == 0 && !getenv("B200_Q3K_GENERIC") && launch_type<T_Q3_K>(W, X, y, y_stride, epi, stream);
     }
     return false;
 }
diff --git a/ggllm.cpp_b200/csrc/mmv_fast.cuh b/ggllm.cpp_b200/csrc/mmv_fast.cuh
--- a/ggllm.cpp_b200/csrc/mmv_fast.cuh
+++ b/ggllm.cpp_b200/csrc/mmv_fast.cuh
@@ -26,7 +26,7 @@
 template <> struct FX<T_Q4_K> {
     static constexpr int PPB = 8;
     static constexpr bool HAS_PROLOGUE_QUANT = true;
-    static constexpr int D256 = 8;
+    static constexpr int NPL = 3;
     struct XR { uint4 xl, xh; int bs; float xd; };
     struct WR { uint4 q; uint32_t sm, dd; };
     __device__ static XR load_x(const int8_t * xq, const ActQ & A, int n, int g) {
@@ -72,18 +72,6 @@
         r.xl = make_uint4(w[0], w[1], w[2], w[3]); r.xh = make_uint4(w[4], w[5], w[6], w[7]);
         r.bs = (s0 & 0xffff) | (s1 << 16);
         (void) lane;
-        return r;
-    }
-    __device__ static WP wp(const WPlanes & W, int g) {
-        WP r; r.b0 = opaque_ptr(W.p[0] + (size_t) g * 16); r.b1 = opaque_ptr(W.p[1] + (size_t) (g >> 1) * 4); r.b2 = opaque_ptr(W.p[2] + (size_t) (g >> 3) * 4);
-        r.s0 = W.stride[0]; r.s1 = W.stride[1]; r.s2 = W.stride[2];
-        return r;
-    }
-    __device__ static WR load_w(const WP & p, uint32_t row) {
-        WR r;
-        r.q = ldg_stream_v4(p.b0 + (uint64_t) row * p.s0);
-        r.sm = ldg_u32(p.b1 + (uint64_t) row * p.s1);
-        r.dd = ldg_u32(p.b2 + (uint64_t) row * p.s2);
         return r;
     }
     __device__ static float dot(const WR & w, const XR & x) {
@@ -99,7 +87,7 @@
 template <> struct FX<T_Q4_0> {
     static constexpr int PPB = 1;
     static constexpr bool HAS_PROLOGUE_QUANT = true;
-    static constexpr int D256 = 8;
+    static constexpr int NPL = 2;
     struct XR { uint4 xl, xh; int bs; float xd; };
     struct WR { uint4 q; uint32_t d; };
     __device__ static XR load_x(const int8_t * xq, const ActQ & A, int n, int g) {
@@ -129,17 +117,6 @@
         }
         r.xl = make_uint4(w[0], w[1], w[2], w[3]); r.xh = make_uint4(w[4], w[5], w[6], w[7]);
         r.bs = s;
-        return r;
-    }
-    __device__ static WP wp(const WPlanes & W, int g) {
-        WP r; r.b0 = opaque_ptr(W.p[0] + (size_t) g * 16); r.b1 = opaque_ptr(W.p[1] + (size_t) g * 2); r.b2 = nullptr;
-        r.s0 = W.stride[0]; r.s1 = W.stride[1]; r.s2 = 0;
-        return r;
-    }
-    __device__ static WR load_w(const WP & p, uint32_t row) {
-        WR r;
-        r.q = ldg_stream_v4(p.b0 + (uint64_t) row * p.s0);
-        r.d = ldg_u16(p.b1 + (uint64_t) row * p.s1);
         return r;
     }
     __device__ static float dot(const WR & w, const XR & x) {
@@ -153,6 +130,7 @@
 template <> struct FX<T_Q3_K> {
     static constexpr int PPB = 4;
     static constexpr bool HAS_PROLOGUE_QUANT = false;
+    static constexpr int NPL = 4;
     static constexpr int D256 = 4;
     struct XR { uint4 x[4]; int bsA, bsB; float xd; };
     struct WR { uint4 q, hm; uint32_t sc, d; };
@@ -235,24 +213,6 @@
 }
 
 
-struct L2PF { const uint8_t * p[3]; uint32_t s[3]; int dist; };
-__device__ __forceinline__ void l2_prefetch_rows(const L2PF & pf, int a, int b) {
-    if (b <= a) return;
-#pragma unroll
-    for (int i = 0; i < 3; i++) {
-        if (!pf.p[i]) continue;
-        const uint8_t * src = pf.p[i] + (size_t) a * pf.s[i];
-        const uint32_t bytes = (uint32_t) (b - a) * pf.s[i];
-        asm volatile("cp.async.bulk.prefetch.L2.global [%0], %1;" :: "l"(src), "r"(bytes) : "memory");
-    }
-}
-__device__ __forceinline__ L2PF l2pf_of(const WPlanes & W, int dist) {
-    L2PF r; r.dist = dist;
-#pragma unroll
-    for (int i = 0; i < 3; i++) { r.p[i] = W.p[i]; r.s[i] = W.stride[i]; }
-    return r;
-}
-
 __device__ __forceinline__ void named_sync(int id, int n) { asm volatile("bar.sync %0, %1;" :: "r"(id), "r"(n) : "memory"); }
 
 template <int TYPE> __device__ __forceinline__ int piece_aux(int g) { return TYPE == T_Q3_K ? 4 * ((g & 3) >> 1) : 0; }
@@ -274,9 +234,8 @@
     }
 }
 
-template <int TYPE, int NTG, int J, int D, bool CHECKED, bool HASNEXT, class Store>
-__device__ __forceinline__ void ring_pass(typename FX<TYPE>::WR (&w)[D][J], const WP (&wp)[J], const int r0, const int nrows, const int npad, const int base,
-                                          const WP (&wpn)[J], const int n0, const int n1,
+template <int TYPE, int NTG, int J, int D, bool CHECKED, class Store>
+__device__ __forceinline__ void ring_pass(typename FX<TYPE>::WR (&w)[D][J], const WP (&wp)[J], const int r0, const int nrows, const int base,
                                           const typename FX<TYPE>::XR (&xr)[J], const int (&aux)[J], float * partial, int & gcount, const int bar_id, const int tg, Store & store) {
     using T = FX<TYPE>;
     constexpr int NWG = NTG / 32, G = (D % 4 == 0) ? 4 : (D % 2 == 0) ? 2 : 1;
@@ -292,10 +251,6 @@
         if (!CHECKED || nxt < nrows) {
 #pragma unroll
             for (int j = 0; j < J; j++) w[s][j] = T::load_w(wp[j], (uint32_t) (r0 + nxt));
-        } else if (HASNEXT && nxt >= npad && n1 > n0) {
-            const uint32_t k = (uint32_t) min(n0 + nxt - npad, n1 - 1);
-#pragma unroll
-            for (int j = 0; j < J; j++) w[s][j] = T::load_w(wpn[j], k);
         }
         if ((s % G) == G - 1) {
             const int gi = (base + s) / G;
@@ -318,19 +273,53 @@
     }
 }
 
-template <int TYPE, int NTG, int J, int D, bool HASNEXT, class Store, class Tail>
+template <int TYPE, int NTG, int J, int D, class Store, class Tail>
 __device__ __forceinline__ void ring_run(typename FX<TYPE>::WR (&w)[D][J], const WP (&wp)[J], const int r0, const int r1,
-                                         const WP (&wpn)[J], const int n0, const int n1,
                                          const typename FX<TYPE>::XR (&xr)[J], const int (&aux)[J], float * partial, int & gcount, const int bar_id, const int tg,
-                                         Store store, Tail before_tail, const L2PF pf = L2PF{ { nullptr, nullptr, nullptr }, { 0, 0, 0 }, 0 }) {
+                                         Store store, Tail before_tail) {
     const int nrows = r1 - r0, npad = (nrows + D - 1) / D * D;
-    if (npad == 0) { before_tail(); if (HASNEXT) ring_fill<TYPE, J, D>(w, wpn, n0, n1); return; }
+    if (npad == 0) { before_tail(); return; }
     int base = 0;
-    for (; base + 2 * D <= nrows; base += D) {
-        if (pf.dist > 0 && tg == 0) l2_prefetch_rows(pf, min(r0 + base + D + pf.dist, r1), min(r0 + base + 2 * D + pf.dist, r1));
-        ring_pass<TYPE, NTG, J, D, false, false>(w, wp, r0, nrows, npad, base, wpn, n0, n1, xr, aux, partial, gcount, bar_id, tg, store);
-    }
+    for (; base + 2 * D <= nrows; base += D)
+        ring_pass<TYPE, NTG, J, D, false>(w, wp, r0, nrows, base, xr, aux, partial, gcount, bar_id, tg, store);
     before_tail();
     for (; base < npad; base += D)
-        ring_pass<TYPE, NTG, J, D, true, HASNEXT>(w, wp, r0, nrows, npad, base, wpn, n0, n1, xr, aux, partial, gcount, bar_id, tg, store);
-}
+        ring_pass<TYPE, NTG, J, D, true>(w, wp, r0, nrows, base, xr, aux, partial, gcount, bar_id, tg, store);
+}
+
+constexpr int RING_MAX_STAGES = 8;
+struct SP { uint32_t o[3], s[3]; };
+
+template <int TYPE> __device__ __forceinline__ SP stage_ptrs(const WPlanes & W, int g, int RS) {
+    SP r;
+    r.s[0] = W.stride[0]; r.s[1] = W.stride[1]; r.s[2] = FX<TYPE>::NPL > 2 ? W.stride[2] : 0;
+    r.o[0] = 16u * g;
+    r.o[1] = RS * r.s[0] + (TYPE == T_Q4_K ? 4u * (g >> 1) : 2u * g);
+    r.o[2] = RS * (r.s[0] + r.s[1]) + 4u * (g >> 3);
+    return r;
+}
+__device__ __forceinline__ uint4 lds_v4(uint32_t a) { uint4 r; asm volatile("ld.shared.v4.u32 {%0,%1,%2,%3}, [%4];" : "=r"(r.x), "=r"(r.y), "=r"(r.z), "=r"(r.w) : "r"(a)); return r; }
+__device__ __forceinline__ uint32_t lds_u32(uint32_t a) { uint32_t r; asm volatile("ld.shared.u32 %0, [%1];" : "=r"(r) : "r"(a)); return r; }
+__device__ __forceinline__ uint32_t lds_u16(uint32_t a) { unsigned short r; asm volatile("ld.shared.u16 %0, [%1];" : "=h"(r) : "r"(a)); return r; }
+
+template <int TYPE> __device__ __forceinline__ typename FX<TYPE>::WR stage_load(uint32_t st, const SP & p, int r) {
+    typename FX<TYPE>::WR w;
+    w.q = lds_v4(st + p.o[0] + r * p.s[0]);
+    if constexpr (TYPE == T_Q4_K) { w.sm = lds_u32(st + p.o[1] + r * p.s[1]); w.dd = lds_u32(st + p.o[2] + r * p.s[2]); }
+    else w.d = lds_u16(st + p.o[1] + r * p.s[1]);
+    return w;
+}
+
+template <int TYPE> __device__ __forceinline__ void stage_issue(const WPlanes & W, uint32_t dst, uint64_t * bar, int row, int nr, int RS) {
+    constexpr int NPL = FX<TYPE>::NPL;
+    uint32_t bytes = 0;
+#pragma unroll
+    for (int i = 0; i < NPL; i++) bytes += (uint32_t) nr * W.stride[i];
+    mbar_expect_tx(bar, bytes);
+#pragma unroll
+    for (int i = 0; i < NPL; i++) {
+        asm volatile("cp.async.bulk.shared::cluster.global.mbarrier::complete_tx::bytes [%0], [%1], %2, [%3];"
+                     :: "r"(dst), "l"(W.p[i] + (size_t) row * W.stride[i]), "r"((uint32_t) nr * W.stride[i]), "r"(smem_u32(bar)) : "memory");
+        dst += (uint32_t) RS * W.stride[i];
+    }
+}
```

Result: slower. 148.6 (median of 6 runs) (-29.8%).
